# lz4/lz4-java

Hardware: AMD Instinct MI355X
Metric: uncompressed GB/s (compress + decompress) per GPU, 64 KiB blocks (higher is better)
Workload: dtype u8; 1 GPU; 65536 x 65536 B blocks per GPU, SURVEY App.F gen_block(seed 0x4C5A3447, litmax 38, win 65535); step = LZ4 fast compress + int32 size gather + LZ4 safe decompress, device-resident; blocks_per_gpu=65536, block_bytes=65536, parallelism=blocks sharded x1

## Files before the change

### lz4-java_amd/csrc/compress_fast.hip

```cpp
#include <hip/hip_runtime.h>
#include <atomic>
#include <cstdio>
#include <cstdlib>
#include <stdint.h>
#include "kernels.h"
#include "kernels_internal.h"
#include "wave_dev.h"
#include "lz4_fast_core.h"
#include "lz4_fast_chain.h"
#include "lz4_fast_ms_core.h"
#include "lz4_fast_v2_core.h"
#include "mail_ring.h"

namespace lz4hip {

#ifndef LZ4HIP_WPC
#define LZ4HIP_WPC 5
#endif
constexpr uint32_t WAVES_PER_CU = LZ4HIP_WPC;
#ifndef LZ4HIP_TABLE_U64
#define LZ4HIP_TABLE_U64 4096
#endif

#ifndef LZ4HIP_MAIL_SLEEP
#define LZ4HIP_MAIL_SLEEP 32
#endif
struct MailDev {
  __device__ __forceinline__ static uint32_t peek(const uint32_t* p) { return __hip_atomic_load(p, __ATOMIC_RELAXED, __HIP_MEMORY_SCOPE_WORKGROUP); }
  __device__ __forceinline__ static uint32_t peek_far(const uint32_t* p) { return __hip_atomic_load(p, __ATOMIC_RELAXED, __HIP_MEMORY_SCOPE_AGENT); }
  __device__ __forceinline__ static void acquire() { __builtin_amdgcn_fence(__ATOMIC_ACQUIRE, "workgroup"); }
  __device__ __forceinline__ static void publish(uint32_t* p, uint32_t v) {
    __builtin_amdgcn_fence(__ATOMIC_RELEASE, "workgroup");
    if (__lane_id() == 0) __hip_atomic_store(p, v, __ATOMIC_RELAXED, __HIP_MEMORY_SCOPE_WORKGROUP);
  }
  __device__ __forceinline__ static void nap_finder() { __builtin_amdgcn_s_sleep(16); }
  __device__ __forceinline__ static void nap_writer() { __builtin_amdgcn_s_sleep(LZ4HIP_MAIL_SLEEP); }
  template <class T> __device__ __forceinline__ static T* uptr(T* q) { return uniform_ptr(q); }
  __device__ __forceinline__ static int32_t u32(int32_t v) { return uniform_i32(v); }
  __device__ __forceinline__ static void block_begin(WaveDev&, const uint8_t*, uint32_t, uint8_t*, uint32_t) {}
  __device__ __forceinline__ static void result(int32_t* out, uint32_t b, int32_t r) { if (__lane_id() == 0) out[b] = r; }
};
template <class W> using MailOut = MailOutT<W, MailDev>;
__device__ __forceinline__ void mail_writer(const BatchArgs& a, uint32_t* slots, uint32_t* ctr) {
  WaveDev w(nullptr);
  mail_writer_t<WaveDev, MailDev>(w, a, slots, ctr);
}

enum : uint32_t { CTL_PK = 0, CTL_OTHER = 1, CTL_DRAW_PK = 2, CTL_WORDS = 64 };
constexpr int32_t PK_MAX_N = 1 << 22;
__device__ __forceinline__ bool pk_block(int32_t n, int32_t cap) { return n >= 65547 && n <= PK_MAX_N && cap >= 0; }
__global__ __launch_bounds__(256) void compress_classify_kernel(const int32_t* src_len, const int32_t* dst_cap, uint32_t n, uint32_t* ctl) {
  const uint32_t i = blockIdx.x * 256u + threadIdx.x;
  const bool in = i < n;
  const bool pk = in && pk_block(src_len[i], dst_cap[i]);
  const uint32_t c_pk = (uint32_t)__builtin_popcountll(__ballot(pk)), c_ot = (uint32_t)__builtin_popcountll(__ballot(in && !pk));
  if (__lane_id() == 0) {
    if (c_pk) atomicAdd(ctl + CTL_PK, c_pk);
    if (c_ot) atomicAdd(ctl + CTL_OTHER, c_ot);
  }
}

__global__ __launch_bounds__(64 * 2 * WAVES_PER_CU) void compress_fast_v2w_cu_kernel(BatchArgs a, uint32_t* q, uint32_t* routed, uint32_t dense64, uint32_t* mail_ctr, uint32_t* mail_slots, const uint32_t* ctl) {
  __shared__ __attribute__((aligned(16))) uint64_t tables[WAVES_PER_CU][LZ4HIP_TABLE_U64];
  const uint32_t wv = threadIdx.x >> 6;
  const uint32_t pair = blockIdx.x * WAVES_PER_CU + (wv < WAVES_PER_CU ? wv : wv - WAVES_PER_CU);
  uint32_t* ctr = mail_ctr + 2u * pair;
  uint32_t* slots = mail_slots + (size_t)pair * (MAIL_RING * MAIL_SLOT_WORDS);
  if (wv >= WAVES_PER_CU) { mail_writer(a, slots, ctr); return; }
  __builtin_amdgcn_s_setprio(3);
  uint64_t* table = tables[wv];
  WaveDev w(table);
  uint32_t head = 0, tail_seen = 0;
  const bool pk_taken = ctl != nullptr && __builtin_amdgcn_readfirstlane(ctl[CTL_PK]) != 0u;
  if (pk_taken && __builtin_amdgcn_readfirstlane(ctl[CTL_OTHER]) == 0u) {
    MailOut<WaveDev> out(w, slots, ctr, head);
    out.post(MAIL_EXIT, 0u, 0u);
    return;
  }
  for (;;) {
    uint32_t b = 0;
    if (__lane_id() == 0) b = atomicAdd(q, 1u);
    b = __builtin_amdgcn_readfirstlane(b);
    if (b < a.n && pk_taken && pk_block(uniform_i32(a.src_len[b]), uniform_i32(a.dst_cap[b]))) continue;
    MailOut<WaveDev> out(w, slots, ctr, head);
    out.tail_seen = tail_seen;
    if (b >= a.n) { out.post(MAIL_EXIT, 0u, 0u); return; }
    out.b = b;
    const int32_t n = uniform_i32(a.src_len[b]);
    const int32_t cap = uniform_i32(a.dst_cap[b]);
    if (n >= 0 && (uint32_t)n <= 0x7E000000u && cap >= 0) {
      const uint8_t* s = uniform_ptr(a.src + a.src_off[b]);
      out.dense64 = routed ? dense64 : 0u;
      if (n < 65547) {
        FastV2<WaveDev, MailOut<WaveDev>> c(w, out, s, (uint32_t)n);
        (void)c.run();
      } else {
        FastV2<WaveDev, MailOut<WaveDev>, false> c(w, out, s, (uint32_t)n);
        (void)c.run();
      }
      if (out.bail) {
        out.post(MAIL_ABORT, 0u, 0u);
        if (__lane_id() == 0) routed[atomicAdd(q + 1, 1u)] = b;
      }
    } else {
      if (__lane_id() == 0) a.out[b] = 0;
    }
    head = out.head; tail_seen = out.tail_seen;
    WaveDev::sync();
  }
}

#ifndef LZ4HIP_PK_FINDERS
#define LZ4HIP_PK_FINDERS 10
#endif
#ifndef LZ4HIP_PK_WRITERS
#define LZ4HIP_PK_WRITERS 6
#endif
#ifndef LZ4HIP_PK_WGS
#define LZ4HIP_PK_WGS 1
#endif
constexpr uint32_t PK_FINDERS = LZ4HIP_PK_FINDERS, PK_WRITERS = LZ4HIP_PK_WRITERS;
constexpr uint32_t PK_WGS_PER_CU = LZ4HIP_PK_WGS;
static_assert(PK_WRITERS <= PK_FINDERS && PK_FINDERS <= 2 * PK_WRITERS && 64 * (PK_FINDERS + PK_WRITERS) <= 1024, "shape of the packed kernel");
__global__ __launch_bounds__(64 * (PK_FINDERS + PK_WRITERS)) void compress_fast_v2wp_cu_kernel(BatchArgs a, uint32_t* ctl, uint32_t* mail_ctr, uint32_t* mail_slots) {
  __shared__ __attribute__((aligned(16))) uint32_t tables[PK_FINDERS][4096];
  if (__builtin_amdgcn_readfirstlane(ctl[CTL_PK]) == 0u) return;
  const uint32_t wv = threadIdx.x >> 6;
  const uint32_t ring0 = blockIdx.x * PK_FINDERS;
  if (wv >= PK_FINDERS) {
    const uint32_t j = wv - PK_FINDERS, k = j + PK_WRITERS;
    WaveDev w(nullptr);
    mail_writer2_t<WaveDev, MailDev>(w, a, mail_slots + (size_t)(ring0 + j) * (MAIL_RING * MAIL_SLOT_WORDS), mail_ctr + 2u * (ring0 + j),
                                     k < PK_FINDERS ? mail_slots + (size_t)(ring0 + k) * (MAIL_RING * MAIL_SLOT_WORDS) : nullptr,
                                     k < PK_FINDERS ? mail_ctr + 2u * (ring0 + k) : nullptr);
    return;
  }
  uint32_t* ctr = mail_ctr + 2u * (ring0 + wv);
  uint32_t* slots = mail_slots + (size_t)(ring0 + wv) * (MAIL_RING * MAIL_SLOT_WORDS);
  __builtin_amdgcn_s_setprio(3);
  WaveDev w((uint64_t*)tables[wv]);
  uint32_t head = 0, tail_seen = 0;
  for (;;) {
    uint32_t b = 0;
    if (__lane_id() == 0) b = atomicAdd(ctl + CTL_DRAW_PK, 1u);
    b = __builtin_amdgcn_readfirstlane(b);
    if (b < a.n && !pk_block(uniform_i32(a.src_len[b]), uniform_i32(a.dst_cap[b]))) continue;
    MailOut<WaveDev> out(w, slots, ctr, head);
    out.tail_seen = tail_seen;
    if (b >= a.n) { out.post(MAIL_EXIT, 0u, 0u); return; }
    out.b = b;
    const int32_t n = uniform_i32(a.src_len[b]);
    const uint8_t* s = uniform_ptr(a.src + a.src_off[b]);
    out.dense64 = 0u;
    {
      FastV2<WaveDev, MailOut<WaveDev>, false, true> c(w, out, s, (uint32_t)n);
      (void)c.run();
    }
    head = out.head; tail_seen = out.tail_seen;
    WaveDev::sync();
  }
}
static std::atomic<int> g_compress_pack{1};
void set_compress_pack(int v) { g_compress_pack.store(v, std::memory_order_relaxed); }
size_t compress_fast_v2w_scratch_words(uint32_t n_cus) {
  const size_t pairs = (size_t)n_cus * (PK_FINDERS * PK_WGS_PER_CU > WAVES_PER_CU ? PK_FINDERS * PK_WGS_PER_CU : WAVES_PER_CU);
  return CTL_WORDS + 2u * pairs + 256u + pairs * (MAIL_RING * MAIL_SLOT_WORDS);
}
int launch_compress_fast_v2w(const BatchArgs& a, uint32_t* q, uint32_t* routed, uint32_t dense64, uint32_t n_cus, uint32_t* mail, void* stream) {
  if (a.n == 0) return 0;
  hipStream_t st = (hipStream_t)stream;
  bool pack = g_compress_pack.load(std::memory_order_relaxed) != 0;
  if (pack) {
    static std::atomic<int> fits[64];
    int d = 0;
    if (hipGetDevice(&d) != hipSuccess || d < 0 || d >= 64) d = 0;
    int f = fits[d].load(std::memory_order_relaxed);
    if (f == 0) {
      int lds = 0;
      f = (hipDeviceGetAttribute(&lds, hipDeviceAttributeMaxSharedMemoryPerBlock, d) == hipSuccess && lds >= 160 * 1024) ? 1 : 2;
      fits[d].store(f, std::memory_order_relaxed);
    }
    if (f != 1) pack = false;
  }
  const size_t pairs_max = (size_t)n_cus * (PK_FINDERS * PK_WGS_PER_CU > WAVES_PER_CU ? PK_FINDERS * PK_WGS_PER_CU : WAVES_PER_CU);
  uint32_t* ctl = mail;
  uint32_t* ctr = mail + CTL_WORDS;
  uint32_t* slots = (uint32_t*)(((uintptr_t)(ctr + 2u * pairs_max) + 1023u) & ~(uintptr_t)1023u);
  hipError_t e = hipMemsetAsync(q, 0, 3 * sizeof(uint32_t), st);
  if (e != hipSuccess) return (int)e;
  e = hipMemsetAsync(mail, 0, (CTL_WORDS + 2u * pairs_max) * sizeof(uint32_t), st);
  if (e != hipSuccess) return (int)e;
  if (pack) {
    if (getenv("LZ4HIP_OCC_DEBUG")) {
      int nb = -1;
      hipError_t oe = hipOccupancyMaxActiveBlocksPerMultiprocessor(&nb, compress_fast_v2wp_cu_kernel, 64 * (PK_FINDERS + PK_WRITERS), 0);
      fprintf(stderr, "[lz4hip] compress_fast_v2wp_cu_kernel: %d workgroups per CU (%s)\n", nb, hipGetErrorString(oe));
    }
    hipLaunchKernelGGL(compress_classify_kernel, dim3((a.n + 255u) / 256u), dim3(256), 0, st, a.src_len, a.dst_cap, a.n, ctl);
    if ((e = hipGetLastError()) != hipSuccess) return (int)e;
    const uint32_t want = (a.n + PK_FINDERS - 1u) / PK_FINDERS, most = n_cus * PK_WGS_PER_CU;
    hipLaunchKernelGGL(compress_fast_v2wp_cu_kernel, dim3(want < most ? want : most), dim3(64 * (PK_FINDERS + PK_WRITERS)), 0, st, a, ctl, ctr, slots);
    if ((e = hipGetLastError()) != hipSuccess) return (int)e;
    e = hipMemsetAsync(ctr, 0, 2u * pairs_max * sizeof(uint32_t), st);
    if (e != hipSuccess) return (int)e;
  }
  const uint32_t wgs = (a.n + WAVES_PER_CU - 1u) / WAVES_PER_CU;
  hipLaunchKernelGGL(compress_fast_v2w_cu_kernel, dim3(wgs < n_cus ? wgs : n_cus), dim3(64 * 2 * WAVES_PER_CU), 0, st, a, q, routed, dense64, ctr, slots,
                     pack ? (const uint32_t*)ctl : (const uint32_t*)nullptr);
  return (int)hipGetLastError();
}

struct BlockIoDev {
  const BatchArgs& a;
  int32_t* consumed = nullptr;
  __device__ __forceinline__ static int32_t i32(int32_t v) { return uniform_i32(v); }
  template <class T> __device__ __forceinline__ static T* ptr(T* p) { return uniform_ptr(p); }
  __device__ __forceinline__ void begin_block(WaveDev&, const uint8_t*, uint32_t, uint8_t*, uint32_t) const {}
  __device__ __forceinline__ void put(uint32_t b, uint32_t r) const { if (__lane_id() == 0) a.out[b] = (int32_t)r; }
  __device__ __forceinline__ void put(uint32_t b, uint32_t r, int32_t c) const { if (__lane_id() == 0) { a.out[b] = (int32_t)r; consumed[b] = c; } }
};
template <class... P, class... A>
static int launch_queue_kernel(void (*kernel)(P...), uint32_t units, uint32_t* q, uint32_t q_words, uint32_t n_cus, void* stream, A... args) {
  if (q_words) {
    hipError_t e = hipMemsetAsync(q, 0, q_words * sizeof(uint32_t), (hipStream_t)stream);
    if (e != hipSuccess) return (int)e;
  }
  const uint32_t wgs = (units + WAVES_PER_CU - 1u) / WAVES_PER_CU;
  hipLaunchKernelGGL(kernel, dim3(wgs < n_cus ? wgs : n_cus), dim3(64 * WAVES_PER_CU), 0, (hipStream_t)stream, args...);
  return (int)hipGetLastError();
}

__global__ __launch_bounds__(64 * WAVES_PER_CU) void compress_fast_ms_cu_kernel(BatchArgs a, uint32_t* q, const uint32_t* routed) {
  __shared__ __attribute__((aligned(16))) uint64_t tables[WAVES_PER_CU][LZ4HIP_TABLE_U64];
  WaveDev w(tables[threadIdx.x >> 6]);
  BlockIoDev io{a};
  const uint32_t count = routed ? __builtin_amdgcn_readfirstlane(q[1]) : a.n;
  for (;;) {
    uint32_t i = 0;
    if (__lane_id() == 0) i = atomicAdd(q + 2, 1u);
    i = __builtin_amdgcn_readfirstlane(i);
    if (i >= count) return;
    FastBlockArgs x;
    fast_block_run<FastFormMS<WaveDev>>(w, io, a, routed ? __builtin_amdgcn_readfirstlane(routed[i]) : i, x);
    WaveDev::sync();
  }
}
int launch_compress_fast_ms(const BatchArgs& a, uint32_t* q, const uint32_t* routed, bool first, uint32_t n_cus, void* stream) {
  if (a.n == 0) return 0;
  return launch_queue_kernel(compress_fast_ms_cu_kernel, a.n, q, first ? 3u : 0u, n_cus, stream, a, q, routed);
}

__global__ __launch_bounds__(64 * WAVES_PER_CU) void compress_fast_accel_cu_kernel(BatchArgs a, uint32_t* q, uint32_t accel) {
  __shared__ __attribute__((aligned(16))) uint64_t tables[WAVES_PER_CU][LZ4HIP_TABLE_U64];
  WaveDev w(tables[threadIdx.x >> 6]);
  BlockIoDev io{a};
  for (;;) {
    uint32_t b = 0;
    if (__lane_id() == 0) b = atomicAdd(q, 1u);
    b = __builtin_amdgcn_readfirstlane(b);
    if (b >= a.n) return;
    FastBlockArgs x;
    x.accel = accel;
    fast_block_run<FastForm<WaveDev, false, true>>(w, io, a, b, x);
    WaveDev::sync();
  }
}
int launch_compress_fast_accel(const BatchArgs& a, uint32_t accel, uint32_t* q, uint32_t n_cus, void* stream) {
  if (a.n == 0) return 0;
  if (accel < 2u || accel > 65537u) return (int)hipErrorInvalidValue;
  return launch_queue_kernel(compress_fast_accel_cu_kernel, a.n, q, 1u, n_cus, stream, a, q, accel);
}

__device__ __forceinline__ void compress_fast_dict_block(const BatchArgs& a, uint32_t b, uint64_t* table, const uint8_t* tail, uint32_t keep,
                                                         const uint8_t* image) {
  const int32_t n = uniform_i32(a.src_len[b]);
  const int32_t cap = uniform_i32(a.dst_cap[b]);
  uint32_t r = 0;
  if (n >= 0 && (uint32_t)n <= 0x7E000000u && cap >= 0) {
    const uint8_t* s = uniform_ptr(a.src + a.src_off[b]);
    uint8_t* d = uniform_ptr(a.dst + a.dst_off[b]);
    WaveDev w(table);
    DirectOut<WaveDev> out(w, s, (uint32_t)n, d, (uint32_t)cap);
    FastCore<WaveDev, false, DirectOut<WaveDev>, false, false, true> c(w, out, s, (uint32_t)n);
    if (keep) { c.dict = tail; c.keep = keep; c.image = image; }
    r = c.run();
  }
  if (__lane_id() == 0) a.out[b] = (int32_t)r;
}
__global__ __launch_bounds__(64 * WAVES_PER_CU) void compress_fast_dict_cu_kernel(BatchArgs a, const uint8_t* tail, uint32_t keep, const uint8_t* image,
                                                                                  uint32_t* q) {
  __shared__ __attribute__((aligned(16))) uint64_t tables[WAVES_PER_CU][LZ4HIP_TABLE_U64];
  uint64_t* table = tables[threadIdx.x >> 6];
  for (;;) {
    uint32_t b = 0;
    if (__lane_id() == 0) b = atomicAdd(q, 1u);
    b = __builtin_amdgcn_readfirstlane(b);
    if (b >= a.n) return;
    compress_fast_dict_block(a, b, table, tail, keep, image);
    WaveDev::sync();
  }
}
int launch_compress_fast_dict(const BatchArgs& a, const uint8_t* dict_end, int32_t keep, const void* image, uint32_t* q, uint32_t n_cus,
                              void* stream) {
  if (a.n == 0) return 0;
  if (keep != 0 && (keep < 8 || keep > 65536 || !dict_end || !image)) return (int)hipErrorInvalidValue;
  return launch_queue_kernel(compress_fast_dict_cu_kernel, a.n, q, 1u, n_cus, stream, a, keep ? dict_end - keep : (const uint8_t*)nullptr,
                             (uint32_t)keep, (const uint8_t*)image, q);
}
__global__ __launch_bounds__(64) void dict_image_kernel(const uint8_t* tail, uint32_t keep, uint8_t* image) {
  __shared__ __attribute__((aligned(16))) uint64_t table[LZ4HIP_TABLE_U64];
  WaveDev w(table);
  dict_image_build(w, tail, keep, image);
}
int launch_dict_image(const uint8_t* tail, int32_t keep, void* image, void* stream) {
  if (keep < 8 || keep > 65536 || !tail || !image) return (int)hipErrorInvalidValue;
  hipLaunchKernelGGL(dict_image_kernel, dim3(1), dim3(64), 0, (hipStream_t)stream, tail, (uint32_t)keep, (uint8_t*)image);
  return (int)hipGetLastError();
}

struct CChainIoDev {
  const CChainArgs& a;
  __device__ __forceinline__ static uint32_t uni(uint32_t v) { return (uint32_t)__builtin_amdgcn_readfirstlane(v); }
  __device__ __forceinline__ static uint64_t uni64(uint64_t v) {
    const uint32_t lo = (uint32_t)__builtin_amdgcn_readfirstlane((uint32_t)v), hi = (uint32_t)__builtin_amdgcn_readfirstlane((uint32_t)(v >> 32));
    return ((uint64_t)hi << 32) | lo;
  }
  template <class T> __device__ __forceinline__ static T* uni_ptr(T* p) { return uniform_ptr(p); }
  __device__ __forceinline__ void put_out(uint32_t i, int32_t r) const { if (__lane_id() == 0) a.out[i] = r; }
  __device__ __forceinline__ void put_chain(uint32_t c, uint64_t n) const { if (__lane_id() == 0) a.chain_consumed[c] = n; }
  __device__ __forceinline__ void begin_block(const uint8_t*, uint32_t, uint8_t*, uint32_t) const {}
};
__global__ __launch_bounds__(64 * WAVES_PER_CU) void compress_fast_chain_cu_kernel(CChainArgs a, uint32_t* q) {
  __shared__ __attribute__((aligned(16))) uint64_t tables[WAVES_PER_CU][LZ4HIP_TABLE_U64];
  WaveDev w(tables[threadIdx.x >> 6]);
  CChainIoDev io{a};
  for (;;) {
    uint32_t c = 0;
    if (__lane_id() == 0) c = atomicAdd(q, 1u);
    c = __builtin_amdgcn_readfirstlane(c);
    if (c >= a.n_chains) return;
    cchain_walk(w, io, a, c);
    WaveDev::sync();
  }
}
int launch_compress_fast_chain(const CChainArgs& a, uint32_t* q, uint32_t n_cus, void* stream) {
  if (a.n_chains == 0) return 0;
  if (!q) return (int)hipErrorInvalidValue;
  return launch_queue_kernel(compress_fast_chain_cu_kernel, a.n_chains, q, 1u, n_cus, stream, a, q);
}

__global__ __launch_bounds__(64 * WAVES_PER_CU) void compress_fast_dest_cu_kernel(BatchArgs a, int32_t* consumed, uint32_t* q) {
  __shared__ __attribute__((aligned(16))) uint64_t tables[WAVES_PER_CU][LZ4HIP_TABLE_U64];
  WaveDev w(tables[threadIdx.x >> 6]);
  BlockIoDev io{a, consumed};
  for (;;) {
    uint32_t b = 0;
    if (__lane_id() == 0) b = atomicAdd(q, 1u);
    b = __builtin_amdgcn_readfirstlane(b);
    if (b >= a.n) return;
    FastBlockArgs x;
    fast_block_run<FastForm<WaveDev, true>>(w, io, a, b, x);
    WaveDev::sync();
  }
}
int launch_compress_dest_size(const BatchArgs& a, int32_t* consumed, uint32_t* q, uint32_t n_cus, void* stream) {
  if (a.n == 0) return 0;
  return launch_queue_kernel(compress_fast_dest_cu_kernel, a.n, q, 1u, n_cus, stream, a, consumed, q);
}

#if LZ4HIP_V2_ASM_PROF
extern "C" __attribute__((visibility("default"))) int lz4hip_dev_asm_prof(unsigned long long* out16) {
  hipError_t e = hipMemcpyFromSymbol(out16, HIP_SYMBOL(g_asm_prof), 16 * sizeof(unsigned long long));
  if (e != hipSuccess) return (int)e;
  unsigned long long z[16] = {0};
  return (int)hipMemcpyToSymbol(HIP_SYMBOL(g_asm_prof), z, sizeof(z));
}
#endif

#if LZ4HIP_ASM_DBG & 4
extern "C" __attribute__((visibility("default"))) int lz4hip_dev_asm_dbg(unsigned int* out1600) {
  return (int)hipMemcpyFromSymbol(out1600, HIP_SYMBOL(g_asm_dbg), 1600 * sizeof(unsigned int));
}
#endif

#ifdef LZ4HIP_DEV_TOOLS
template <int MS>
__global__ __launch_bounds__(64) void compress_fast_prof_kernel(BatchArgs a, uint64_t* prof) {
  __shared__ __attribute__((aligned(16))) uint64_t table[4096];
  const uint32_t b = blockIdx.x;
  const int32_t n = a.src_len[b];
  const int32_t cap = a.dst_cap[b];
  uint32_t r = 0;
  FastStats st = {};
  if (n >= 0 && (uint32_t)n <= 0x7E000000u && cap >= 0) {
    const uint8_t* s = a.src + a.src_off[b];
    uint8_t* d = a.dst + a.dst_off[b];
    WaveDev w(table);
    DirectOut<WaveDev> out(w, s, (uint32_t)n, d, (uint32_t)cap);
    if constexpr (MS == 3) {
      ParkOutRaw<WaveDev> po(w, s, (uint32_t)n, d, (uint32_t)cap);
      if (n < 65547) { FastV2<WaveDev, ParkOutRaw<WaveDev>> c(w, po, s, (uint32_t)n, &st); r = c.run(); }
      else { FastV2<WaveDev, ParkOutRaw<WaveDev>, false> c(w, po, s, (uint32_t)n, &st); r = c.run(); }
    } else if constexpr (MS == 1) {
      if (n < 65547) { FastCoreMS<WaveDev, true> c(w, out, s, (uint32_t)n, &st); r = c.run(); }
      else { FastCoreMS<WaveDev, false> c(w, out, s, (uint32_t)n, &st); r = c.run(); }
    } else {
      if (n < 65547) { FastCore<WaveDev, true> c(w, out, s, (uint32_t)n, &st); r = c.run(); }
      else { FastCore<WaveDev, false> c(w, out, s, (uint32_t)n, &st); r = c.run(); }
    }
  }
  if (threadIdx.x == 0) {
    a.out[b] = (int32_t)r;
    uint64_t* p = prof + (uint64_t)b * 12u;
    p[0] = st.steps; p[1] = st.slow_steps; p[2] = st.false_pos; p[3] = st.sequences;
    for (int i = 0; i < 8; i++) p[4 + i] = st.t[i];
  }
}
int launch_compress_fast_prof(const BatchArgs& a, uint64_t* prof, int core, void* stream) {
  if (a.n == 0) return 0;
  if (core == 3) hipLaunchKernelGGL(compress_fast_prof_kernel<3>, dim3(a.n), dim3(64), 0, (hipStream_t)stream, a, prof);
  else if (core >= 1) hipLaunchKernelGGL(compress_fast_prof_kernel<1>, dim3(a.n), dim3(64), 0, (hipStream_t)stream, a, prof);
  else hipLaunchKernelGGL(compress_fast_prof_kernel<0>, dim3(a.n), dim3(64), 0, (hipStream_t)stream, a, prof);
  return (int)hipGetLastError();
}
#endif

}
```

### lz4-java_amd/csrc/lz4_fast_v2_core.h

```cpp
#pragma once
#include "lz4_fast_core.h"
#if defined(__HIPCC__)
#include "lz4_fast_v2_asm.h"
#include "lz4_fast_v2_asm32.h"
#endif

#ifndef LZ4HIP_V2_PROBE
#define LZ4HIP_V2_PROBE 0
#endif

namespace lz4hip {

LZ4HIP_DEV int ctz32(uint32_t x) { return __builtin_ctz(x); }
LZ4HIP_DEV int clz64(uint64_t x) { return __builtin_clzll(x); }

template <class W>
struct ParkOut {
  using VU = typename W::VU;
  using VU64 = typename W::VU64;
  using VB = typename W::VB;
  static constexpr bool kUsesWindowRegs = false;
  static constexpr uint32_t kNoCheck = 1u << 16;
  static constexpr uint32_t kFinal = 1u << 17;
  static constexpr bool kRawPark = false;
  static constexpr bool kAsmPark = false;

  W& w;
  const uint8_t* src;
  uint32_t n;
  uint8_t* dst;
  uint32_t cap;
  bool limited;
  uint32_t op = 0;
  VU p_ms, p_ml, p_off;
  uint32_t cnt = 0;
  uint32_t prev_end = 0;
  bool ok = true;
  uint32_t dense64 = 0, flushes = 0, mark = 0;
  bool bail = false;

  LZ4HIP_DEV ParkOut(W& w_, const uint8_t* s, uint32_t n_, uint8_t* d, uint32_t cap_) : w(w_), src(s), n(n_), dst(d), cap(cap_) {
    limited = cap < n + n / 255u + 16u;
    p_ms = VU(0u); p_ml = VU(0u); p_off = VU(0u);
  }

  LZ4HIP_DEV static uint32_t ext_count(uint32_t len) { return len >= 15u ? (len - 15u) / 255u + 1u : 0u; }
  LZ4HIP_DEV void put_ext(uint32_t o, uint32_t len, uint32_t c) {
    const uint32_t rem = (len - 15u) - 255u * (c - 1u);
    for (uint32_t base = 0; base < c; base += 64u) {
      VU i = w.lane() + base;
      w.st8(dst, i + o, W::select(i == c - 1u, VU(rem), VU(255u)), i < c);
    }
  }

  LZ4HIP_DEV void park(uint32_t ms, uint32_t ml, uint32_t offx) {
    p_ms = W::writelane(p_ms, ms, cnt);
    p_ml = W::writelane(p_ml, ml, cnt);
    p_off = W::writelane(p_off, offx, cnt);
    if (++cnt == 64u) flush();
  }

  LZ4HIP_DEV void resolve_raw() {
    if (cnt == 0u) return;
    const VU j = w.lane();
    const VB act = j < cnt;
    const VB raw = act & ((p_off & kFinal) == 0u);
    const VU endv = p_ms + p_ml;
    const VU anchor = W::select(j == 0u, VU(prev_end), W::shfl_up1(endv));
    const VU off = p_off & 0xFFFFu;
    const VU mpos = p_ms - off;
    const VU room = p_ms - anchor;
    const VU maxback = W::vmin(room, mpos);
    VU back = VU(0u);
    VB go = raw & (maxback > 0u);
    while (w.ballot(go)) {
      const VU a = w.ld8(src, p_ms - 1u - back, go), b = w.ld8(src, mpos - 1u - back, go);
      const VB eq = go & (a == b);
      back = W::select(eq, back + 1u, back);
      go = eq & (back < maxback);
    }
    p_ms = p_ms - back;
    p_ml = p_ml + back;
    p_off = W::select(raw, off | W::select(room == 0u, VU(kNoCheck), VU(0u)), p_off & ~kFinal);
  }

  LZ4HIP_DEV void flush() {
    if (cnt == 0u) return;
    const uint32_t m = cnt;
    cnt = 0u;
    if (!ok) return;
    const VU j = w.lane();
    const VB act = j < m;
    const VU endv = p_ms + p_ml;
    const VU anchor = W::select(j == 0u, VU(prev_end), W::shfl_up1(endv));
    const VU lit = p_ms - anchor;
    const VU mc = p_ml - 4u;
    const VU offset = p_off & 0xFFFFu;
    const VU nlx = W::select(lit >= 15u, W::div255(lit - 15u) + 1u, VU(0u));
    const VU nmx = W::select(mc >= 15u, W::div255(mc - 15u) + 1u, VU(0u));
    const VU size = W::select(act, nlx + lit + nmx + 3u, VU(0u));
    const VU o = w.excl_scan(size) + op;
    const uint32_t end = w.bcast(o + size, (int)(m - 1u));
    prev_end = w.bcast(endv, (int)(m - 1u));
    if (dense64 != 0u && flushes < 2u && m == 64u) {
      const uint32_t e31 = w.bcast(endv, 31);
      if (flushes == 0u) mark = e31;
      else if (e31 - mark < dense64) { bail = true; return; }
      flushes++;
    }
    if (limited) {
      const VB c1 = ((p_off & kNoCheck) == 0u) & (W::u64(o) + W::u64(lit) + W::u64(W::div255(lit)) + VU64(1u + 8u) > VU64((uint64_t)cap));
      const VB c2 = W::u64(o) + W::u64(nlx) + W::u64(lit) + W::u64(W::div255(mc + 240u)) + VU64(1u + 2u + 6u) > VU64((uint64_t)cap);
      if (w.ballot(act & (c1 | c2))) { ok = false; return; }
    }
    const VU ld = o + nlx + 1u;
    uint32_t i = 0;
    for (; i < 48u; i += 16u) {
      if (!w.ballot(act & (VU(i + 4u) <= lit))) break;
      VU t[4];
      VB mk[4];
#pragma unroll
      for (uint32_t k = 0; k < 4u; k++) { mk[k] = act & (VU(i + 4u * k + 4u) <= lit); t[k] = w.ld32(src, anchor + (i + 4u * k), mk[k]); }
#pragma unroll
      for (uint32_t k = 0; k < 4u; k++) w.st32(dst, ld + (i + 4u * k), t[k], mk[k]);
    }
    for (;; i += 4u) {
      const VB mk = act & (VU(i + 4u) <= lit);
      if (!w.ballot(mk)) break;
      w.st32(dst, ld + i, w.ld32(src, anchor + i, mk), mk);
    }
    {
      const VU t0 = lit & ~3u;
      VU tb[3];
      VB mk[3];
#pragma unroll
      for (uint32_t k = 0; k < 3u; k++) { mk[k] = act & (t0 + k < lit); tb[k] = w.ld8(src, anchor + t0 + k, mk[k]); }
#pragma unroll
      for (uint32_t k = 0; k < 3u; k++) w.st8(dst, ld + t0 + k, tb[k], mk[k]);
    }
    const VU tok = (W::vmin(lit, VU(15u)) << 4) | W::vmin(mc, VU(15u));
    w.st8(dst, o, tok, act);
    w.st8(dst, o + 1u, lit - 15u, act & (nlx == 1u));
    const VU oo = ld + lit;
    w.st8(dst, oo, offset & 0xFFu, act);
    w.st8(dst, oo + 1u, offset >> 8, act);
    w.st8(dst, oo + 2u, mc - 15u, act & (nmx == 1u));
    uint64_t longs = w.ballot(act & ((nlx > 1u) | (nmx > 1u)));
    while (longs) {
      const int k = ctz64(longs);
      longs &= longs - 1u;
      const uint32_t l = w.bcast(lit, k), c = w.bcast(mc, k), ok_ = w.bcast(o, k), nl = w.bcast(nlx, k), nm = w.bcast(nmx, k);
      if (nl > 1u) put_ext(ok_ + 1u, l, nl);
      if (nm > 1u) put_ext(ok_ + 1u + nl + l + 2u, c, nm);
    }
    op = end;
  }

  LZ4HIP_DEV uint32_t emit_last(uint32_t anchor) {
    const uint32_t last = n - anchor;
    if (limited && (uint64_t)op + last + 1u + (last + 255u - 15u) / 255u > cap) return 0;
    const uint32_t nlx = ext_count(last);
    w.st8(dst, VU(op), VU((last < 15u ? last : 15u) << 4), w.lane() == 0u);
    if (nlx) put_ext(op + 1u, last, nlx);
    w.copy(dst, op + 1u + nlx, src, anchor, last);
    return op + 1u + nlx + last;
  }

  LZ4HIP_DEV bool overlap_point() { return ok; }
  LZ4HIP_DEV void seq(uint32_t lit, uint32_t mc, uint32_t offset, uint32_t anchor, bool check_lits, bool, VU) {
    park(anchor + lit, mc + 4u, offset | (check_lits ? 0u : kNoCheck));
  }
  LZ4HIP_DEV uint32_t last(uint32_t anchor) {
    flush();
    if (!ok) return 0u;
    return emit_last(anchor);
  }
};

template <class W>
struct ParkOutRaw : ParkOut<W> {
  using P = ParkOut<W>;
  using VU = typename W::VU;
  static constexpr bool kRawPark = true;
  LZ4HIP_DEV ParkOutRaw(W& w_, const uint8_t* s, uint32_t n_, uint8_t* d, uint32_t cap_) : P(w_, s, n_, d, cap_) {}
  LZ4HIP_DEV void park(uint32_t ms, uint32_t ml, uint32_t offx) {
    P::p_ms = W::writelane(P::p_ms, ms, P::cnt);
    P::p_ml = W::writelane(P::p_ml, ml, P::cnt);
    P::p_off = W::writelane(P::p_off, offx, P::cnt);
    if (++P::cnt == 64u) { P::resolve_raw(); P::flush(); }
  }
  LZ4HIP_DEV bool overlap_point() { return P::ok; }
  LZ4HIP_DEV void seq(uint32_t lit, uint32_t mc, uint32_t offset, uint32_t anchor, bool check_lits, bool, VU) {
    park(anchor + lit, mc + 4u, offset | (check_lits ? 0u : P::kNoCheck) | P::kFinal);
  }
  LZ4HIP_DEV uint32_t last(uint32_t anchor) {
    P::resolve_raw();
    return P::last(anchor);
  }
};

template <class W, class OUT = ParkOut<W>, bool U16 = true, bool PK = false>
struct FastV2 {
  using VU = typename W::VU;
  using VU64 = typename W::VU64;
  using VB = typename W::VB;
  using Gen = FastCore<W, U16, OUT, PK>;
  static constexpr bool S32 = Gen::S32;
  using VE = typename Gen::VE;
  using E = typename Gen::E;
  static constexpr uint32_t kFwdBytes = 256u;
  static constexpr uint32_t kTail = 12u + 64u + kFwdBytes + 16u;

  W& w;
  OUT& out;
  const uint8_t* src;
  uint32_t n;
  FastStats* st;

  LZ4HIP_DEV FastV2(W& w_, OUT& out_, const uint8_t* s, uint32_t n_, FastStats* st_ = nullptr) : w(w_), out(out_), src(s), n(n_), st(st_) {}

  LZ4HIP_DEV uint32_t run() {
    if (n < 13u) return out.last(0u);
    {
      const uint32_t x0 = w.sld32(src, 0);
      if constexpr (U16) w.template lds_fill<true>(1u << Gen::HLOG, (((x0 * 2654435761u) >> 3) & LZ4HIP_FP_MASK));
      else w.template lds_fill<S32>(1u << Gen::HLOG, (E)(((x0 * 2654435761u) >> 16) & Gen::FPM));
      w.sync();
    }
    Gen gen(w, out, src, n, st);
#if defined(__HIP_DEVICE_COMPILE__) && LZ4HIP_V2_ASM_PROF
    const uint64_t prof_t0 = w.tick(n);
    uint64_t prof_lean = 0, prof_calls = 0;
#endif
    uint32_t r = gen.template loop<2>(false, 1u, 0u, 0u);
    while (gen.one_done && !out.bail) {
      gen.one_done = false;
#if defined(__HIP_DEVICE_COMPILE__) && LZ4HIP_V2_ASM_PROF
      const uint64_t prof_l0 = w.tick(gen.p_ip);
      const uint32_t ip = lean(gen.p_ip);
      prof_lean += w.tick(ip) - prof_l0; prof_calls++;
#else
      const uint32_t ip = lean(gen.p_ip);
#endif
      gen.anchor = ip;
      const uint64_t tx = st ? w.tick(ip) : 0;
      r = gen.template loop<2>(true, ip + 1u, 0u, ip);
      if (st) { st->t[6] += w.tick(r) - tx; st->t[7] += 1; }
    }
#if defined(__HIP_DEVICE_COMPILE__) && LZ4HIP_V2_ASM_PROF
    if (w.lane() == 0u) {
      for (int i = 0; i < 6; i++) atomicAdd(&g_asm_prof[i], (unsigned long long)aprof[i]);
      atomicAdd(&g_asm_prof[6], (unsigned long long)prof_lean);
      atomicAdd(&g_asm_prof[7], (unsigned long long)(w.tick(r) - prof_t0));
      atomicAdd(&g_asm_prof[8], 1ull);
      atomicAdd(&g_asm_prof[9], (unsigned long long)prof_calls);
    }
#endif
    return r;
  }

  uint32_t aprof[8] = {0, 0, 0, 0, 0, 0, 0, 0};
  LZ4HIP_DEV uint32_t lean(uint32_t ip) {
    if (n < kTail + 8u) return ip;
    const uint32_t lim = n - kTail;
    const VU j = w.lane();
    const VU cj = W::select(j == 0u, VU(0xFFFFFFFEu), j - 1u);
    const VU j4 = j * 4u;
    uint32_t pf_end = ip & ~(W::kPrefetchBytes - 1u);
    uint64_t l_steps = 0, l_slow = 0, l_seq = 0, l_t[6] = {0, 0, 0, 0, 0, 0}, tk_keep = 0;
    VU prev_fa = VU(0u);
    uint32_t prev_hpos = 0x80000000u;
    while (ip <= lim && !out.bail) {
#if defined(__HIP_DEVICE_COMPILE__) && LZ4HIP_V2_ASM
#ifndef LZ4HIP_V2_ROWLOAD
#define LZ4HIP_V2_ROWLOAD 1
#endif
      if constexpr (LZ4HIP_V2_ROWLOAD && W::kAsmLean && OUT::kAsmPark) {
        if (!st && ip - prev_hpos > (U16 ? 127u : 126u) && ip >= 2u && out.cnt < 63u) {
          prev_hpos = ip - 2u;
          prev_fa = w.ldu32(src, j4 + prev_hpos);
        }
      }
      if constexpr (U16 && W::kAsmLean && OUT::kAsmPark) {
        if (!st) {
#if LZ4HIP_ASM_DBG & 4
          const uint32_t dbg_ip = ip, dbg_pc = out.cnt, dbg_php = prev_hpos;
#endif
          if (__builtin_amdgcn_read_exec() != ~0ull) __builtin_trap();
          const uint32_t code = lean_asm_run(ip, prev_hpos, pf_end, out.cnt, prev_fa, out.p_ms, out.p_ml, out.p_off,
                                             lim >= 192u ? lim - 192u : 0u, src,
                                             (uint32_t)(uintptr_t)(__attribute__((address_space(3))) char*)w.lds, n, aprof);
#if LZ4HIP_ASM_DBG & 4
          if (w.lane() == 0u) {
            const unsigned long long k = atomicAdd(&g_asm_prof[15], 1ull);
            if (k < 200) { g_asm_dbg[k * 8 + 0] = dbg_ip; g_asm_dbg[k * 8 + 1] = dbg_php; g_asm_dbg[k * 8 + 2] = dbg_pc; g_asm_dbg[k * 8 + 3] = code;
                           g_asm_dbg[k * 8 + 4] = ip; g_asm_dbg[k * 8 + 5] = prev_hpos; g_asm_dbg[k * 8 + 6] = out.cnt; g_asm_dbg[k * 8 + 7] = 0; }
          }
#endif
          (void)code;
          if (out.cnt == 64u) { out.batch(); continue; }
          if (ip > lim) break;
        }
      }
#ifndef LZ4HIP_V2_ASM32
#define LZ4HIP_V2_ASM32 1
#endif
      if constexpr (!U16 && LZ4HIP_V2_ASM32 && !LZ4HIP_V2_ASM_PROF && W::kAsmLean && OUT::kAsmPark) {
        if (!st) {
          if (__builtin_amdgcn_read_exec() != ~0ull) __builtin_trap();
          if constexpr (PK)
            (void)lean_asm_run32p(ip, prev_hpos, pf_end, out.cnt, prev_fa, out.p_ms, out.p_ml, out.p_off,
                                  lim >= 192u ? lim - 192u : 0u, src,
                                  (uint32_t)(uintptr_t)(__attribute__((address_space(3))) char*)w.lds, n);
          else
          (void)lean_asm_run32(ip, prev_hpos, pf_end, out.cnt, prev_fa, out.p_ms, out.p_ml, out.p_off,
                               lim >= 192u ? lim - 192u : 0u, src,
                               (uint32_t)(uintptr_t)(__attribute__((address_space(3))) char*)w.lds, n);
          if (out.cnt == 64u) { out.batch(); continue; }
          if (ip > lim) break;
        }
      }
#elif defined(LZ4HIP_HOST_ASM_EMU)
      if constexpr (W::kAsmLean && OUT::kAsmPark) {
        if (!st) {
          if (ip - prev_hpos > (U16 ? 127u : 126u) && ip >= 2u && out.cnt < 63u) {
            prev_hpos = ip - 2u;
            prev_fa = w.ldu32(src, j4 + prev_hpos);
          }
          w.template lean_asm_emu<U16, PK>(ip, prev_hpos, pf_end, out.cnt, prev_fa, out.p_ms, out.p_ml, out.p_off, lim >= 192u ? lim - 192u : 0u, src, n);
          if (out.cnt == 64u) { out.batch(); continue; }
          if (ip > lim) break;
        }
      }
#endif
      if (st) l_steps++;
      uint64_t tk = (st && LZ4HIP_V2_PROBE == 0) ? w.tick(ip) : tk_keep;
#define LZ4HIP_PHASE2(i, dep) do { if (st) { if (LZ4HIP_V2_PROBE == 0) { const uint64_t t_ = w.tick(dep); l_t[i] += t_ - tk; tk = t_; } \
        else if (LZ4HIP_V2_PROBE == (i) + 2 || (LZ4HIP_V2_PROBE == 1 && (i) == 5)) { tk_keep = tk = w.tick(dep); } \
        else if (LZ4HIP_V2_PROBE == (i) + 1) { l_t[i] += w.tick(dep) - tk; } } } while (0)
      const VU pos = cj + ip;
#ifndef LZ4HIP_V2_WIN_FROM_ROW
#define LZ4HIP_V2_WIN_FROM_ROW 1
#endif
      VU x32, x32b = VU(0u);
      if (LZ4HIP_V2_WIN_FROM_ROW && LZ4HIP_LIKELY(ip - prev_hpos <= (U16 ? 189u : 185u))) {
        const VU o = cj + (ip - prev_hpos);
        const VU d = o >> 2;
        const VU w1 = W::shfl(prev_fa, d + 1u);
        x32 = W::alignbyte(w1, W::shfl(prev_fa, d), o & 3u);
        if constexpr (!U16) x32b = W::alignbyte(W::shfl(prev_fa, d + 2u), w1, o & 3u);
      } else {
        if constexpr (U16) x32 = w.ldu32(src, pos);
        else { const VU64 x64 = w.ldu64(src, pos); x32 = W::lo32(x64); x32b = W::lo32(x64 >> 32); }
      }
      VU h, fp;
      if constexpr (U16) {
        const VU prod = x32 * 2654435761u;
        h = prod >> (32 - Gen::HLOG);
        fp = (prod >> 3) & LZ4HIP_FP_MASK;
      } else {
        const VU64 x64 = W::u64(x32) | (W::u64(x32b) << 32);
        h = W::lo32(((x64 << 24) * 889523592379ull) >> (64 - Gen::HLOG));
        fp = Gen::fp32(x32);
      }
      LZ4HIP_PHASE2(0, w.bcast(h, 0));
      const VE e = w.template lds_rdu<S32>(h);
      const VE newe = Gen::mk_entry(pos, fp);
      uint64_t tmask = w.ballot(Gen::e_fp(e) == fp) & ~1ull;
      if constexpr (!U16) tmask &= w.ballot(Gen::e_pos(e) + Gen::MAXD >= pos);
#ifndef LZ4HIP_COUNT_CAT
#define LZ4HIP_COUNT_CAT 5
#endif
      if (LZ4HIP_UNLIKELY(tmask == 0)) { if (st && LZ4HIP_COUNT_CAT == 5) st->false_pos++; break; }
      LZ4HIP_PHASE2(1, (uint32_t)tmask);
#ifndef LZ4HIP_V2_PVERIFY
#define LZ4HIP_V2_PVERIFY 0
#endif
      VU c4 = VU(0u);
      if (LZ4HIP_V2_PVERIFY && OUT::kRawPark) c4 = w.ld32(src, Gen::e_pos(e), w.lanes(tmask & (tmask - 1ull)));
      uint64_t tm = tmask;
      uint32_t lo = 0;
      uint32_t k0, hpos, mpos, cnt;
      uint64_t upto;
      VU fa, bb = VU(0u);
      VB bval = VB(false);
      bool fail = false;
      for (;;) {
        k0 = (uint32_t)ctz64(tm);
        upto = (2ull << k0) - 1ull;
        const uint64_t inm = upto & ~((1ull << lo) - 1ull);
        const VE old = w.template lds_max<S32>(h, newe, w.lanes(inm));
        hpos = ip + k0 - 1u;
        mpos = Gen::se_pos(w.template bcast_e<S32>(e, (int)k0));
        fa = w.ldu32(src, j4 + hpos);
        const VU fb = w.ldu32(src, j4 + mpos);
        if constexpr (!OUT::kRawPark) {
          const VU bidx = j + (mpos - k0);
          bval = j + mpos >= VU(k0);
          bb = w.ldu8(src, W::select(bval, bidx, VU(0u)));
        }
        if (LZ4HIP_UNLIKELY(hpos + W::kPrefetchBytes > pf_end)) {
          if (pf_end < n) w.prefetch4k(src, pf_end, n);
          pf_end += W::kPrefetchBytes;
        }
        LZ4HIP_PHASE2(2, mpos);
        const uint64_t det = w.ballot(old != e) & inm;
        LZ4HIP_PHASE2(3, (uint32_t)det);
        const VU fx = fa ^ fb;
        const uint64_t dm = w.ballot(fx != 0u);
        cnt = 0;
        if (LZ4HIP_LIKELY(dm != 0)) {
          const int f = ctz64(dm);
          cnt = 4u * (uint32_t)f + ((uint32_t)ctz32(w.bcast(fx, f)) >> 3);
        }
        LZ4HIP_PHASE2(4, cnt);
        bool bad = dm == 0;
        bool ruled_out = dm != 0 && cnt < 4u;
        if (LZ4HIP_UNLIKELY(det != 0)) {
          if (det & (det - 1u)) {
            bad = true;
            if (st && LZ4HIP_COUNT_CAT == 1) st->false_pos++;
          } else {
            const int dl = ctz64(det);
            const uint32_t od = w.bcast(Gen::e_fp(old), dl), hd = w.bcast(h, dl), fd = w.bcast(fp, dl);
            if (od == fd) { bad = true; if (st && LZ4HIP_COUNT_CAT == 2) st->false_pos++; }
            else if (hd == w.bcast(h, (int)k0)) ruled_out = true;
          }
        }
        if (st && LZ4HIP_COUNT_CAT == 3 && dm == 0) st->false_pos++;
        if (st && LZ4HIP_COUNT_CAT == 4 && !bad && ruled_out && (tm & ~upto) == 0) st->false_pos++;
        if (LZ4HIP_LIKELY(!bad && !ruled_out)) break;
        if (OUT::kRawPark && !bad) {
          tm &= ~upto;
          if (LZ4HIP_V2_PVERIFY) tm &= w.ballot(c4 == x32);
          lo = k0 + 1u;
          if (tm) continue;
        }
        if (st) l_slow++;
        w.template lds_wr<S32>(h, e, w.lanes(upto));
        w.sync();
        fail = true;
        break;
      }
      if (LZ4HIP_UNLIKELY(fail)) break;
      w.sync();
      if (st) l_seq++;
      if constexpr (OUT::kRawPark) {
        out.park(hpos, cnt, hpos - mpos);
      } else {
        const uint64_t eqm = w.ballot(bval & ((x32 & 0xFFu) == bb));
        const uint64_t range = ((1ull << k0) - 1ull) & ~1ull;
        const uint64_t ne = (~eqm & range) | 1ull;
        const uint32_t back = k0 - 1u - (63u - (uint32_t)clz64(ne));
        out.park(hpos - back, cnt + back, (hpos - mpos) | (k0 == 1u ? OUT::kNoCheck : 0u));
      }
      ip = hpos + cnt;
      prev_fa = fa;
      prev_hpos = hpos;
      LZ4HIP_PHASE2(5, ip);
    }
#undef LZ4HIP_PHASE2
    if (st) { st->steps += l_steps; st->slow_steps += l_slow; st->sequences += l_seq; for (int i = 0; i < 6; i++) st->t[i] += l_t[i]; }
    return ip;
  }
};

}
```

Baseline: 101.6 GB/s.

## Finish block tail with a single chained loop and align lean asm entry

```diff
diff --git a/lz4-java_amd/csrc/compress_fast.hip b/lz4-java_amd/csrc/compress_fast.hip
--- a/lz4-java_amd/csrc/compress_fast.hip
+++ b/lz4-java_amd/csrc/compress_fast.hip
@@ -71,6 +71,9 @@
   uint64_t* table = tables[wv];
   WaveDev w(table);
   uint32_t head = 0, tail_seen = 0;
+#if LZ4HIP_V2_ASM_PROF
+  uint64_t prof_mark = WaveDev::tick(wv);
+#endif
   const bool pk_taken = ctl != nullptr && __builtin_amdgcn_readfirstlane(ctl[CTL_PK]) != 0u;
   if (pk_taken && __builtin_amdgcn_readfirstlane(ctl[CTL_OTHER]) == 0u) {
     MailOut<WaveDev> out(w, slots, ctr, head);
@@ -91,6 +94,9 @@
     if (n >= 0 && (uint32_t)n <= 0x7E000000u && cap >= 0) {
       const uint8_t* s = uniform_ptr(a.src + a.src_off[b]);
       out.dense64 = routed ? dense64 : 0u;
+#if LZ4HIP_V2_ASM_PROF
+      { const uint64_t t_ = WaveDev::tick((uint32_t)(uintptr_t)s); if (__lane_id() == 0) atomicAdd(&g_replay_prof[10], (unsigned long long)(t_ - prof_mark)); }
+#endif
       if (n < 65547) {
         FastV2<WaveDev, MailOut<WaveDev>> c(w, out, s, (uint32_t)n);
         (void)c.run();
@@ -107,6 +113,9 @@
     }
     head = out.head; tail_seen = out.tail_seen;
     WaveDev::sync();
+#if LZ4HIP_V2_ASM_PROF
+    prof_mark = WaveDev::tick(head);
+#endif
   }
 }
 
@@ -374,6 +383,12 @@
   if (e != hipSuccess) return (int)e;
   unsigned long long z[16] = {0};
   return (int)hipMemcpyToSymbol(HIP_SYMBOL(g_asm_prof), z, sizeof(z));
+}
+extern "C" __attribute__((visibility("default"))) int lz4hip_dev_replay_prof(unsigned long long* out16) {
+  hipError_t e = hipMemcpyFromSymbol(out16, HIP_SYMBOL(g_replay_prof), 16 * sizeof(unsigned long long));
+  if (e != hipSuccess) return (int)e;
+  unsigned long long z[16] = {0};
+  return (int)hipMemcpyToSymbol(HIP_SYMBOL(g_replay_prof), z, sizeof(z));
 }
 #endif
 
diff --git a/lz4-java_amd/csrc/lz4_fast_v2_core.h b/lz4-java_amd/csrc/lz4_fast_v2_core.h
--- a/lz4-java_amd/csrc/lz4_fast_v2_core.h
+++ b/lz4-java_amd/csrc/lz4_fast_v2_core.h
@@ -5,11 +5,27 @@
 #include "lz4_fast_v2_asm32.h"
 #endif
 
+#ifndef LZ4HIP_V2_ASM_PAD
+#define LZ4HIP_V2_ASM_PAD 4
+#endif
+#ifndef LZ4HIP_V2_ASM32_PAD
+#define LZ4HIP_V2_ASM32_PAD 6
+#endif
+#ifndef LZ4HIP_V2_ASM32P_PAD
+#define LZ4HIP_V2_ASM32P_PAD 4
+#endif
+#if defined(__HIP_DEVICE_COMPILE__)
+#define LZ4HIP_LEAN_ALIGN(pad) asm volatile("  s_branch L_lean_al_%=\n  .p2align 6\n  .rept " LZ4HIP_STR(pad) "\n  s_nop 0\n  .endr\nL_lean_al_%=:\n" : : :)
+#endif
 #ifndef LZ4HIP_V2_PROBE
 #define LZ4HIP_V2_PROBE 0
 #endif
 
 namespace lz4hip {
+
+#if defined(__HIPCC__) && LZ4HIP_V2_ASM_PROF
+__device__ unsigned long long g_replay_prof[16];
+#endif
 
 LZ4HIP_DEV int ctz32(uint32_t x) { return __builtin_ctz(x); }
 LZ4HIP_DEV int clz64(uint64_t x) { return __builtin_clzll(x); }
@@ -205,6 +221,9 @@
   using VU64 = typename W::VU64;
   using VB = typename W::VB;
   using Gen = FastCore<W, U16, OUT, PK>;
+#ifndef LZ4HIP_V2_TAIL_CHAIN
+#define LZ4HIP_V2_TAIL_CHAIN 1
+#endif
   static constexpr bool S32 = Gen::S32;
   using VE = typename Gen::VE;
   using E = typename Gen::E;
@@ -219,8 +238,13 @@
 
   LZ4HIP_DEV FastV2(W& w_, OUT& out_, const uint8_t* s, uint32_t n_, FastStats* st_ = nullptr) : w(w_), out(out_), src(s), n(n_), st(st_) {}
 
+  uint32_t tail_chains = 0;
+
   LZ4HIP_DEV uint32_t run() {
     if (n < 13u) return out.last(0u);
+#if defined(__HIP_DEVICE_COMPILE__) && LZ4HIP_V2_ASM_PROF
+    const uint64_t prof_f0 = w.tick(n);
+#endif
     {
       const uint32_t x0 = w.sld32(src, 0);
       if constexpr (U16) w.template lds_fill<true>(1u << Gen::HLOG, (((x0 * 2654435761u) >> 3) & LZ4HIP_FP_MASK));
@@ -230,23 +254,37 @@
     Gen gen(w, out, src, n, st);
 #if defined(__HIP_DEVICE_COMPILE__) && LZ4HIP_V2_ASM_PROF
     const uint64_t prof_t0 = w.tick(n);
-    uint64_t prof_lean = 0, prof_calls = 0;
-#endif
-    uint32_t r = gen.template loop<2>(false, 1u, 0u, 0u);
-    while (gen.one_done && !out.bail) {
-      gen.one_done = false;
+    uint64_t prof_lean = 0, prof_calls = 0, prof_exact = 0, prof_tail = 0;
+#define LZ4HIP_RUN_PROF(acc, dep, ...) do { const uint64_t t_ = w.tick(dep); __VA_ARGS__; acc += w.tick(r) - t_; } while (0)
+#else
+#define LZ4HIP_RUN_PROF(acc, dep, ...) do { __VA_ARGS__; } while (0)
+#endif
+    const bool lean_runs = n >= kTail + 8u;
+    uint32_t r = 0u, ip = 0u;
+    bool chain = LZ4HIP_V2_TAIL_CHAIN && !lean_runs, post = false;
+    if (!chain) {
+      LZ4HIP_RUN_PROF(prof_exact, n, r = gen.template loop<2>(false, 1u, 0u, 0u));
+      while (gen.one_done && !out.bail) {
+        gen.one_done = false;
 #if defined(__HIP_DEVICE_COMPILE__) && LZ4HIP_V2_ASM_PROF
-      const uint64_t prof_l0 = w.tick(gen.p_ip);
-      const uint32_t ip = lean(gen.p_ip);
-      prof_lean += w.tick(ip) - prof_l0; prof_calls++;
+        const uint64_t prof_l0 = w.tick(gen.p_ip);
+        ip = lean(gen.p_ip);
+        prof_lean += w.tick(ip) - prof_l0; prof_calls++;
 #else
-      const uint32_t ip = lean(gen.p_ip);
-#endif
-      gen.anchor = ip;
-      const uint64_t tx = st ? w.tick(ip) : 0;
-      r = gen.template loop<2>(true, ip + 1u, 0u, ip);
-      if (st) { st->t[6] += w.tick(r) - tx; st->t[7] += 1; }
-    }
+        ip = lean(gen.p_ip);
+#endif
+        gen.anchor = ip;
+        if (LZ4HIP_V2_TAIL_CHAIN && lean_runs && ip > n - kTail) { chain = post = true; break; }
+        const uint64_t tx = st ? w.tick(ip) : 0;
+        LZ4HIP_RUN_PROF(prof_exact, ip, r = gen.template loop<2>(true, ip + 1u, 0u, ip));
+        if (st) { st->t[6] += w.tick(r) - tx; st->t[7] += 1; }
+      }
+    }
+    if (chain) {
+      tail_chains++;
+      LZ4HIP_RUN_PROF(prof_tail, ip, r = gen.template loop<0>(post, ip + 1u, 0u, ip));
+    }
+#undef LZ4HIP_RUN_PROF
 #if defined(__HIP_DEVICE_COMPILE__) && LZ4HIP_V2_ASM_PROF
     if (w.lane() == 0u) {
       for (int i = 0; i < 6; i++) atomicAdd(&g_asm_prof[i], (unsigned long long)aprof[i]);
@@ -254,12 +292,15 @@
       atomicAdd(&g_asm_prof[7], (unsigned long long)(w.tick(r) - prof_t0));
       atomicAdd(&g_asm_prof[8], 1ull);
       atomicAdd(&g_asm_prof[9], (unsigned long long)prof_calls);
+      const unsigned long long v[10] = {prof_exact, prof_tail, prof_t0 - prof_f0, rprof[0], rprof[1], rprof[2], rprof[3], rprof[4], rprof[5], rprof[6]};
+      for (int i = 0; i < 10; i++) atomicAdd(&g_replay_prof[i], v[i]);
     }
 #endif
     return r;
   }
 
   uint32_t aprof[8] = {0, 0, 0, 0, 0, 0, 0, 0};
+  uint64_t rprof[8] = {0, 0, 0, 0, 0, 0, 0, 0};
   LZ4HIP_DEV uint32_t lean(uint32_t ip) {
     if (n < kTail + 8u) return ip;
     const uint32_t lim = n - kTail;
@@ -287,6 +328,9 @@
           const uint32_t dbg_ip = ip, dbg_pc = out.cnt, dbg_php = prev_hpos;
 #endif
           if (__builtin_amdgcn_read_exec() != ~0ull) __builtin_trap();
+#if LZ4HIP_V2_ASM_PAD >= 0
+          LZ4HIP_LEAN_ALIGN(LZ4HIP_V2_ASM_PAD);
+#endif
           const uint32_t code = lean_asm_run(ip, prev_hpos, pf_end, out.cnt, prev_fa, out.p_ms, out.p_ml, out.p_off,
                                              lim >= 192u ? lim - 192u : 0u, src,
                                              (uint32_t)(uintptr_t)(__attribute__((address_space(3))) char*)w.lds, n, aprof);
@@ -298,6 +342,11 @@
           }
 #endif
           (void)code;
+#if LZ4HIP_V2_ASM_PROF
+          rprof[2]++;
+          if (out.cnt == 64u) rprof[3]++;
+          if (out.cnt == 64u) { const uint64_t t_ = w.tick(ip); out.batch(); rprof[0] += w.tick(out.cnt) - t_; continue; }
+#endif
           if (out.cnt == 64u) { out.batch(); continue; }
           if (ip > lim) break;
         }
@@ -308,14 +357,21 @@
       if constexpr (!U16 && LZ4HIP_V2_ASM32 && !LZ4HIP_V2_ASM_PROF && W::kAsmLean && OUT::kAsmPark) {
         if (!st) {
           if (__builtin_amdgcn_read_exec() != ~0ull) __builtin_trap();
-          if constexpr (PK)
+          if constexpr (PK) {
+#if LZ4HIP_V2_ASM32P_PAD >= 0
+            LZ4HIP_LEAN_ALIGN(LZ4HIP_V2_ASM32P_PAD);
+#endif
             (void)lean_asm_run32p(ip, prev_hpos, pf_end, out.cnt, prev_fa, out.p_ms, out.p_ml, out.p_off,
                                   lim >= 192u ? lim - 192u : 0u, src,
                                   (uint32_t)(uintptr_t)(__attribute__((address_space(3))) char*)w.lds, n);
-          else
-          (void)lean_asm_run32(ip, prev_hpos, pf_end, out.cnt, prev_fa, out.p_ms, out.p_ml, out.p_off,
-                               lim >= 192u ? lim - 192u : 0u, src,
-                               (uint32_t)(uintptr_t)(__attribute__((address_space(3))) char*)w.lds, n);
+          } else {
+#if LZ4HIP_V2_ASM32_PAD >= 0
+            LZ4HIP_LEAN_ALIGN(LZ4HIP_V2_ASM32_PAD);
+#endif
+            (void)lean_asm_run32(ip, prev_hpos, pf_end, out.cnt, prev_fa, out.p_ms, out.p_ml, out.p_off,
+                                 lim >= 192u ? lim - 192u : 0u, src,
+                                 (uint32_t)(uintptr_t)(__attribute__((address_space(3))) char*)w.lds, n);
+          }
           if (out.cnt == 64u) { out.batch(); continue; }
           if (ip > lim) break;
         }
@@ -334,6 +390,13 @@
       }
 #endif
       if (st) l_steps++;
+#if defined(__HIP_DEVICE_COMPILE__) && LZ4HIP_V2_ASM_PROF
+      const uint64_t prof_c0 = w.tick(ip);
+      rprof[4]++;
+#define LZ4HIP_CSTEP_END(k, dep) do { rprof[1] += w.tick(dep) - prof_c0; if (k) rprof[k]++; } while (0)
+#else
+#define LZ4HIP_CSTEP_END(k, dep) do { } while (0)
+#endif
       uint64_t tk = (st && LZ4HIP_V2_PROBE == 0) ? w.tick(ip) : tk_keep;
 #define LZ4HIP_PHASE2(i, dep) do { if (st) { if (LZ4HIP_V2_PROBE == 0) { const uint64_t t_ = w.tick(dep); l_t[i] += t_ - tk; tk = t_; } \
         else if (LZ4HIP_V2_PROBE == (i) + 2 || (LZ4HIP_V2_PROBE == 1 && (i) == 5)) { tk_keep = tk = w.tick(dep); } \
@@ -371,7 +434,7 @@
 #ifndef LZ4HIP_COUNT_CAT
 #define LZ4HIP_COUNT_CAT 5
 #endif
-      if (LZ4HIP_UNLIKELY(tmask == 0)) { if (st && LZ4HIP_COUNT_CAT == 5) st->false_pos++; break; }
+      if (LZ4HIP_UNLIKELY(tmask == 0)) { if (st && LZ4HIP_COUNT_CAT == 5) st->false_pos++; LZ4HIP_CSTEP_END(5, ip); break; }
       LZ4HIP_PHASE2(1, (uint32_t)tmask);
 #ifndef LZ4HIP_V2_PVERIFY
 #define LZ4HIP_V2_PVERIFY 0
@@ -442,7 +505,7 @@
         fail = true;
         break;
       }
-      if (LZ4HIP_UNLIKELY(fail)) break;
+      if (LZ4HIP_UNLIKELY(fail)) { LZ4HIP_CSTEP_END(6, ip); break; }
       w.sync();
       if (st) l_seq++;
       if constexpr (OUT::kRawPark) {
@@ -458,7 +521,9 @@
       prev_fa = fa;
       prev_hpos = hpos;
       LZ4HIP_PHASE2(5, ip);
-    }
+      LZ4HIP_CSTEP_END(0, ip);
+    }
+#undef LZ4HIP_CSTEP_END
 #undef LZ4HIP_PHASE2
     if (st) { st->steps += l_steps; st->slow_steps += l_slow; st->sequences += l_seq; for (int i = 0; i < 6; i++) st->t[i] += l_t[i]; }
     return ip;
```

Result: no change. 102.4 GB/s (median of 6 runs) (+0.8%).
